# chansoopark98/Deep-Visual-SLAM

Hardware: AMD Instinct MI355X
Metric: VO training-step frames/sec (3-frame 640x480 snippets) (higher is better)
Workload: dtype f32; 1 GPU; configs[2]/[3]: full 4-scale photometric+smoothness loss, batch 12 per GPU, ResNet-18; per_gpu_batch=12, global_batch=12, num_scales=4, image=640x480, parallelism=dp1, streams=depth | pose | 2x weight-gradient, optimizer=fused Adam pass at lr 0: every step computes from the seeded weights, gpu_max_hw_queues=4

## Files before the change

deep-visual-slam_amd/csrc/conv_thin.hip:

```cpp
#include "conv_common.h"

#include <cstdlib>
#include <type_traits>

#ifndef THIN_DBG
#define THIN_DBG 0
#endif

namespace dvsconv {
namespace {

struct ThinParams {
    const float* x;
    const float* x2;
    const float* dy;
    const float* y;
    float* dw;
    float* dbias;
    int B, H, W, C1, C2, up, dact;
    int nseg, rows_per_wg, row_chunks;
};

template <int MT>
struct Acc {
    using type = typename std::conditional<MT == 32, f32x16, f32x4>::type;
};

template <int I, int N, class F>
__device__ __forceinline__ void static_for_thin(F&& f) {
    if constexpr (I < N) {
        f(std::integral_constant<int, I>{});
        static_for_thin<I + 1, N>(f);
    }
}

__device__ __forceinline__ f32x16 mma(float a, float b, f32x16 c) { return __builtin_amdgcn_mfma_f32_32x32x2f32(a, b, c, 0, 0, 0); }
__device__ __forceinline__ f32x4 mma(float a, float b, f32x4 c) { return __builtin_amdgcn_mfma_f32_16x16x4f32(a, b, c, 0, 0, 0); }

template <int MT, int CIN, int SEG>
__global__ __launch_bounds__(NT) void thin_wgrad_kernel(ThinParams p) {
    constexpr int KS = 64 / MT;
    constexpr int CT = CIN / MT;
    constexpr int NTILE = 9 * CT;
    constexpr int PWAVES = (MT == 16) ? 4 : 1;
    constexpr int TWAVES = 4 / PWAVES;
    constexpr int TPW = (NTILE + TWAVES - 1) / TWAVES;
    constexpr int PXW = SEG / PWAVES;
    constexpr int STEPS = PXW / KS;
    constexpr int CS = (MT == 16 && CIN % 32 == 0) ? CIN + 16 : CIN;
    constexpr int COLS = SEG + 2;
    constexpr int ROWF = COLS * CS;
    constexpr int XV = CIN / 4, ROW_VECS = COLS * XV, X_LOADS = (ROW_VECS + NT - 1) / NT;
    constexpr int DV = MT / 4, D_VECS = SEG * DV, D_LOADS = (D_VECS + NT - 1) / NT;
    static_assert(CIN % MT == 0 && SEG % (PWAVES * KS) == 0 && D_VECS % 64 == 0, "shape");
    using acc_t = typename Acc<MT>::type;
    constexpr int NR = (MT == 32) ? 16 : 4;

    __shared__ __attribute__((aligned(16))) float Ps[4 * ROWF];
    __shared__ __attribute__((aligned(16))) float Ds[2][SEG][MT];

    const int tid = threadIdx.x, lane = tid & 63;
    const int wave = __builtin_amdgcn_readfirstlane(tid >> 6);
    const int pw = wave / TWAVES, tw = wave % TWAVES;
    int lg = xcd_logical(blockIdx.x, gridDim.x, 1);
    const int chunk = lg % p.row_chunks;
    lg /= p.row_chunks;
    const int seg = lg % p.nseg, b = lg / p.nseg;
    const int oy_begin = chunk * p.rows_per_wg, oy_end = min(p.H, oy_begin + p.rows_per_wg);
    const int x0 = seg * SEG;
    const int Cout = MT, Ktot = 9 * CIN;
    const int H1 = p.up ? p.H >> 1 : p.H, W1 = p.up ? p.W >> 1 : p.W;

    int x_goff[X_LOADS], x_loff[X_LOADS];
    bool x_ok[X_LOADS], x_is2[X_LOADS];
#pragma unroll
    for (int j = 0; j < X_LOADS; ++j) {
        const int idx = tid + NT * j;
        x_ok[j] = idx < ROW_VECS;
        const int px = min(idx, ROW_VECS - 1) / XV, c = (min(idx, ROW_VECS - 1) % XV) * 4;
        const int sx = reflect_i(x0 - 1 + px, p.W);
        x_is2[j] = c >= p.C1;
        x_goff[j] = x_is2[j] ? sx * p.C2 + (c - p.C1) : (p.up ? sx >> 1 : sx) * p.C1 + c;
        x_loff[j] = px * CS + c;
    }
#ifdef THIN_NS
    constexpr int NS = THIN_NS;
#else
    constexpr int NS = 2;
#endif
    f32x4 rx[NS > 3 ? NS : 3][X_LOADS];
    auto load_row = [&](int pr, auto set) {
        constexpr int S = decltype(set)::value;
        const int sr = reflect_i(min(pr, p.H + 1) - 1, p.H);
        const float* r1 = p.x + ((size_t)b * H1 + (p.up ? sr >> 1 : sr)) * W1 * p.C1;
        const float* r2 = p.C2 > 0 ? p.x2 + ((size_t)b * p.H + sr) * p.W * p.C2 : r1;
#pragma unroll
        for (int j = 0; j < X_LOADS; ++j) rx[S][j] = *reinterpret_cast<const f32x4*>((x_is2[j] ? r2 : r1) + x_goff[j]);
    };
    auto store_row = [&](int pr, auto set) {
        constexpr int S = decltype(set)::value;
        float* dst = Ps + (pr & 3) * ROWF;
#pragma unroll
        for (int j = 0; j < X_LOADS; ++j)
            if (x_ok[j]) *reinterpret_cast<f32x4*>(dst + x_loff[j]) = rx[S][j];
    };

    f32x4 rd[NS][D_LOADS], ry[NS][D_LOADS], bsum = {0.f, 0.f, 0.f, 0.f};
    const int d_c = (tid % DV) * 4;
    const bool d_ok = tid < D_VECS;
    auto load_d = [&](int oy, auto set) {
        constexpr int S = decltype(set)::value;
        if (d_ok) {
#pragma unroll
            for (int j = 0; j < D_LOADS; ++j) {
                const size_t o = (((size_t)b * p.H + min(oy, p.H - 1)) * p.W + x0 + (tid + NT * j) / DV) * Cout + d_c;
                rd[S][j] = *reinterpret_cast<const f32x4*>(p.dy + o);
                if (p.dact) ry[S][j] = *reinterpret_cast<const f32x4*>(p.y + o);
            }
        }
    };
    auto store_d = [&](int buf, auto set) {
        constexpr int S = decltype(set)::value;
        if (d_ok) {
#pragma unroll
            for (int j = 0; j < D_LOADS; ++j) {
                f32x4 v = rd[S][j];
                if (p.dact == ACT_ELU) {
#pragma unroll
                    for (int e = 0; e < 4; ++e) v[e] = fmaf(v[e], fminf(ry[S][j][e], 0.f), v[e]);
                } else if (p.dact) {
#pragma unroll
                    for (int e = 0; e < 4; ++e) v[e] *= act_grad_from_out(ry[S][j][e], p.dact);
                }
                *reinterpret_cast<f32x4*>(&Ds[buf][(tid + NT * j) / DV][d_c]) = v;
                bsum += v;
            }
        }
    };

    const int col = lane % MT, kidx = lane / MT;
    int t_ky[TPW], t_off[TPW];
    bool t_ok[TPW];
#pragma unroll
    for (int i = 0; i < TPW; ++i) {
        const int q = tw + TWAVES * i;
        t_ok[i] = q < NTILE;
        const int qq = t_ok[i] ? q : 0;
        const int tap = qq / CT, ct = qq % CT;
        t_ky[i] = tap / 3;
        t_off[i] = (tap % 3) * CS + ct * MT;
    }
    const int b_lane = (pw * PXW + kidx) * CS + col;
    const int a_lane = (pw * PXW + kidx) * MT + col;

    acc_t acc[TPW];
#pragma unroll
    for (int i = 0; i < TPW; ++i)
#pragma unroll
        for (int r = 0; r < NR; ++r) acc[i][r] = 0.f;

    using S0 = std::integral_constant<int, 0>;
    if (oy_begin < oy_end) {
        static_for_thin<0, 3>([&](auto k) { load_row(oy_begin + k.value, k); });
        load_d(oy_begin, S0{});
        static_for_thin<0, 3>([&](auto k) { store_row(oy_begin + k.value, k); });
        store_d(0, S0{});
        static_for_thin<0, NS - 1>([&](auto k) {
            load_row(oy_begin + 3 + k.value, k);
            load_d(oy_begin + 1 + k.value, k);
        });
        for (int i = tid; i < ROWF; i += NT) Ps[((oy_begin + 3) & 3) * ROWF + i] = 0.f;
        for (int i = tid; i < SEG * MT; i += NT) (&Ds[1][0][0])[i] = 0.f;
    }
    __syncthreads();
    int buf = 0;
    auto stage = [&](int oy, auto set) {
        constexpr int S = decltype(set)::value;
        using Free = std::integral_constant<int, (S + NS - 1) % NS>;
        const bool more = oy + 1 < oy_end;
        if (oy + NS < oy_end && !(THIN_DBG & 1)) {
            load_row(oy + 2 + NS, Free{});
            load_d(oy + NS, Free{});
        }
        const float* Ab = &Ds[buf][0][0] + a_lane;
        const float* Bb[TPW];
#pragma unroll
        for (int i = 0; i < TPW; ++i) Bb[i] = Ps + ((oy + t_ky[i]) & 3) * ROWF + t_off[i] + b_lane;
        const float live = oy < oy_end ? 1.f : 0.f;
        float aq[2], bq[2][TPW];
        aq[0] = Ab[0];
#pragma unroll
        for (int i = 0; i < TPW; ++i) bq[0][i] = Bb[i][0];
#pragma unroll
        for (int t = 0; t < STEPS; ++t) {
            if (t + 1 < STEPS) {
                aq[(t + 1) & 1] = Ab[(t + 1) * KS * MT];
#pragma unroll
                for (int i = 0; i < TPW; ++i) bq[(t + 1) & 1][i] = Bb[i][(t + 1) * KS * CS];
            }
            __builtin_amdgcn_sched_barrier(0);
            const float a = aq[t & 1] * live;
            if constexpr (THIN_DBG & 2) {
#pragma unroll
                for (int i = 0; i < TPW; ++i) acc[i][0] += a * bq[t & 1][i];
            } else {
#pragma unroll
                for (int i = 0; i < TPW; ++i) acc[i] = mma(a, bq[t & 1][i], acc[i]);
            }
            __builtin_amdgcn_sched_barrier(0);
        }
        if (more && !(THIN_DBG & 4)) {
            store_row(oy + 3, set);
            store_d(buf ^ 1, set);
        }
        if (!(THIN_DBG & 8)) __syncthreads();
        buf ^= 1;
    };
#pragma unroll 1
    for (int oy = oy_begin; oy < oy_end; oy += NS) static_for_thin<0, NS>([&](auto k) { stage(oy + k.value, k); });

    if constexpr (PWAVES > 1) {
        static_assert(Cout * 9 * CIN <= 4 * ROWF, "dW fits the ring");
        float* sw = Ps;
        for (int i = tid; i < Cout * Ktot; i += NT) sw[i] = 0.f;
        __syncthreads();
#pragma unroll
        for (int i = 0; i < TPW; ++i) {
            if (!t_ok[i]) continue;
            const int q = tw + TWAVES * i;
            const int kk = (q / CT) * CIN + (q % CT) * MT + col;
#pragma unroll
            for (int r = 0; r < NR; ++r) atomicAdd(sw + (4 * (lane >> 4) + r) * Ktot + kk, acc[i][r]);
        }
        __syncthreads();
        constexpr int NW = Cout * 9 * CIN;
        const int rot = (int)((blockIdx.x * 7u) % (unsigned)(NW / NT)) * NT;
        for (int i = tid; i < NW; i += NT) {
            const int j = i + rot < NW ? i + rot : i + rot - NW;
            atomicAdd(p.dw + j, sw[j]);
        }
    } else {
#pragma unroll
        for (int i = 0; i < TPW; ++i) {
            if (!t_ok[i]) continue;
            const int q = tw + TWAVES * i;
            const int kk = (q / CT) * CIN + (q % CT) * MT + col;
#pragma unroll
            for (int r = 0; r < NR; ++r) {
                const int co = (MT == 32) ? (r & 3) + 8 * (r >> 2) + 4 * (lane >> 5) : 4 * (lane >> 4) + r;
                atomicAdd(p.dw + (size_t)co * Ktot + kk, acc[i][r]);
            }
        }
    }
    if (p.dbias) {
        float* sb = &Ds[0][0][0];
        if (tid < MT) sb[tid] = 0.f;
        __syncthreads();
        if (d_ok) {
#pragma unroll
            for (int e = 0; e < 4; ++e) atomicAdd(&sb[d_c + e], bsum[e]);
        }
        __syncthreads();
        if (tid < MT) atomicAdd(p.dbias + tid, sb[tid]);
    }
}

template <int MT, int CIN, int SEG>
void launch_thin(ThinParams p, hipStream_t st) {
    p.nseg = p.W / SEG;
    static const int slots = [] {
        int occ = 0, dev = 0, cus = 256;
        hipGetDevice(&dev);
        hipDeviceGetAttribute(&cus, hipDeviceAttributeMultiprocessorCount, dev);
        if (hipOccupancyMaxActiveBlocksPerMultiprocessor(&occ, thin_wgrad_kernel<MT, CIN, SEG>, NT, 0) != hipSuccess || occ < 1) occ = 1;
        return cus * occ;
    }();
    const int cols = p.B * p.nseg;
    int chunks = max(1, min(slots / cols, p.H / 8));
    p.rows_per_wg = (p.H + chunks - 1) / chunks;
    p.row_chunks = (p.H + p.rows_per_wg - 1) / p.rows_per_wg;
    dvs::ProfScope prof(dvs::SLOT_CONV_WGRAD, st);
    prof.work(2.0 * p.B * p.H * p.W * MT * 9.0 * CIN);
    hipLaunchKernelGGL((thin_wgrad_kernel<MT, CIN, SEG>), dim3(cols * p.row_chunks), dim3(NT), 0, st, p);
}


struct ThinFwdParams {
    const float* x;
    const float* w;
    const float* bias;
    float* y;
    int B, H, W, up, act;
    int nseg, rows_per_wg, row_chunks;
};

__device__ __forceinline__ float thin_act(float v, int act) {
    switch (act) {
        case ACT_RELU: return fmaxf(v, 0.f);
        case ACT_ELU: return v > 0.f ? v : __expf(v) - 1.f;
        case ACT_SIGMOID: return 1.f / (1.f + __expf(-v));
        default: return v;
    }
}

template <int CIN, int SEG>
__global__ __launch_bounds__(NT) void thin_fwd_kernel(ThinFwdParams p) {
    constexpr int CO = 16;
    constexpr int CS = CIN + 2;
    constexpr int COLS = SEG + 2, ROWF = COLS * CS;
    constexpr int XV = CIN / 4, ROW_VECS = COLS * XV, X_LOADS = (ROW_VECS + NT - 1) / NT;
    constexpr int PXW = SEG / 4, PT = PXW / 16;
    constexpr int C4 = CIN / 4, KSTEPS = 9 * C4;
    static_assert(PXW % 16 == 0 && (ROWF % 2) == 0, "shape");
    __shared__ __attribute__((aligned(16))) float Ps[4 * ROWF];

    const int tid = threadIdx.x, lane = tid & 63;
    const int wave = __builtin_amdgcn_readfirstlane(tid >> 6);
    int lg = xcd_logical(blockIdx.x, gridDim.x, 1);
    const int chunk = lg % p.row_chunks;
    lg /= p.row_chunks;
    const int seg = lg % p.nseg, b = lg / p.nseg;
    const int oy_begin = chunk * p.rows_per_wg, oy_end = min(p.H, oy_begin + p.rows_per_wg);
    const int x0 = seg * SEG;
    const int H1 = p.up ? p.H >> 1 : p.H, W1 = p.up ? p.W >> 1 : p.W;

    int x_goff[X_LOADS], x_loff[X_LOADS];
    bool x_ok[X_LOADS];
#pragma unroll
    for (int j = 0; j < X_LOADS; ++j) {
        const int idx = tid + NT * j;
        x_ok[j] = idx < ROW_VECS;
        const int px = min(idx, ROW_VECS - 1) / XV, c = (min(idx, ROW_VECS - 1) % XV) * 4;
        const int sx = reflect_i(x0 - 1 + px, p.W);
        x_goff[j] = (p.up ? sx >> 1 : sx) * CIN + c;
        x_loff[j] = px * CS + c;
    }
    f32x4 rx[X_LOADS];
    auto load_row_to = [&](int pr, f32x4 (&r)[X_LOADS]) {
        const int sr = reflect_i(pr - 1, p.H);
        const float* r1 = p.x + ((size_t)b * H1 + (p.up ? sr >> 1 : sr)) * W1 * CIN;
#pragma unroll
        for (int j = 0; j < X_LOADS; ++j) r[j] = *reinterpret_cast<const f32x4*>(r1 + x_goff[j]);
    };
    auto store_row_from = [&](int pr, const f32x4 (&r)[X_LOADS]) {
        float* dst = Ps + (pr & 3) * ROWF;
#pragma unroll
        for (int j = 0; j < X_LOADS; ++j)
            if (x_ok[j]) {
                float2* d2 = reinterpret_cast<float2*>(dst + x_loff[j]);
                d2[0] = float2{r[j][0], r[j][1]};
                d2[1] = float2{r[j][2], r[j][3]};
            }
    };
    auto load_row = [&](int pr) { load_row_to(pr, rx); };
    auto store_row = [&](int pr) { store_row_from(pr, rx); };

    const int n = lane & 15, kidx = lane >> 4;
    float wreg[KSTEPS];
#pragma unroll
    for (int s = 0; s < KSTEPS; ++s) wreg[s] = p.w[(size_t)n * (9 * CIN) + (s / C4) * CIN + (s % C4) * 4 + kidx];
    const float bv = p.bias ? p.bias[n] : 0.f;
    const int a_lane = (wave * PXW + n) * CS + kidx;

    if (oy_begin < oy_end) {
        f32x4 r0[X_LOADS], r1[X_LOADS];
        load_row_to(oy_begin, r0);
        load_row_to(oy_begin + 1, r1);
        load_row(oy_begin + 2);
        store_row_from(oy_begin, r0);
        store_row_from(oy_begin + 1, r1);
        store_row(oy_begin + 2);
    }
    __syncthreads();
#pragma unroll 1
    for (int oy = oy_begin; oy < oy_end; ++oy) {
        const bool more = oy + 1 < oy_end;
        if (more) load_row(oy + 3);
        const float* Ar[3];
#pragma unroll
        for (int ky = 0; ky < 3; ++ky) Ar[ky] = Ps + ((oy + ky) & 3) * ROWF + a_lane;
        f32x4 acc[PT];
#pragma unroll
        for (int t = 0; t < PT; ++t) acc[t] = f32x4{0.f, 0.f, 0.f, 0.f};
#pragma unroll
        for (int s = 0; s < KSTEPS; ++s) {
            const int tap = s / C4, c4 = s % C4, ky = tap / 3, kx = tap % 3;
#pragma unroll
            for (int t = 0; t < PT; ++t) acc[t] = mma(Ar[ky][(t * 16 + kx) * CS + c4 * 4], wreg[s], acc[t]);
        }
        float* yrow = p.y + (((size_t)b * p.H + oy) * p.W + x0 + wave * PXW + 4 * kidx) * CO + n;
#pragma unroll
        for (int t = 0; t < PT; ++t)
#pragma unroll
            for (int r = 0; r < 4; ++r) yrow[(t * 16 + r) * CO] = thin_act(acc[t][r] + bv, p.act);
        if (more) store_row(oy + 3);
        __syncthreads();
    }
}

template <int CIN, int SEG>
void launch_thin_fwd(ThinFwdParams p, hipStream_t st) {
    p.nseg = p.W / SEG;
    static const int slots = [] {
        int occ = 0, dev = 0, cus = 256;
        hipGetDevice(&dev);
        hipDeviceGetAttribute(&cus, hipDeviceAttributeMultiprocessorCount, dev);
        if (hipOccupancyMaxActiveBlocksPerMultiprocessor(&occ, thin_fwd_kernel<CIN, SEG>, NT, 0) != hipSuccess || occ < 1) occ = 1;
        return cus * occ;
    }();
    const int cols = p.B * p.nseg;
    int chunks = max(1, min(slots / cols, p.H / 8));
    p.rows_per_wg = (p.H + chunks - 1) / chunks;
    p.row_chunks = (p.H + p.rows_per_wg - 1) / p.rows_per_wg;
    dvs::ProfScope prof(dvs::SLOT_CONV_FWD, st);
    prof.work(2.0 * p.B * p.H * p.W * 16 * 9.0 * CIN);
    hipLaunchKernelGGL((thin_fwd_kernel<CIN, SEG>), dim3(cols * p.row_chunks), dim3(NT), 0, st, p);
}


struct ThinDgradParams {
    const float* dy;
    const float* y;
    const float* wt;
    float* dx;
    float* dx_skip;
    int B, H, W, dact, nout, C1;
    int nseg, rows_per_wg, row_chunks, nsplit;
};

template <int CK, int NTN, int SEG>
__device__ __forceinline__ void thin_dgrad_body(const ThinDgradParams& p) {
    constexpr int CS = CK + 2, C4 = CK / 4;
    constexpr int COLS = SEG + 2, ROWF = COLS * CS;
    constexpr int ROW_VECS = COLS * C4, X_LOADS = (ROW_VECS + NT - 1) / NT;
    constexpr int PXW = SEG / 4, PT = PXW / 16;
    static_assert(PXW % 16 == 0, "shape");
    __shared__ __attribute__((aligned(16))) float Ps[4 * ROWF];

    const int tid = threadIdx.x, lane = tid & 63;
    const int wave = __builtin_amdgcn_readfirstlane(tid >> 6);
    int lg = xcd_logical(blockIdx.x, gridDim.x, 1);
    const int split = lg % p.nsplit;
    lg /= p.nsplit;
    const int chunk = lg % p.row_chunks;
    lg /= p.row_chunks;
    const int seg = lg % p.nseg, b = lg / p.nseg;
    const int iy_begin = chunk * p.rows_per_wg, iy_end = min(p.H, iy_begin + p.rows_per_wg);
    const int x0 = seg * SEG;
    const int n_base = split * 16 * NTN;
    bool coarse[NTN];
    bool any_coarse = false, any_direct = false;
#pragma unroll
    for (int nt = 0; nt < NTN; ++nt) {
        coarse[nt] = n_base + nt * 16 < p.C1;
        any_coarse = any_coarse || coarse[nt];
        any_direct = any_direct || !coarse[nt];
    }

    int x_goff[X_LOADS], x_loff[X_LOADS];
    bool x_ok[X_LOADS], x_in[X_LOADS];
#pragma unroll
    for (int j = 0; j < X_LOADS; ++j) {
        const int idx = tid + NT * j;
        x_ok[j] = idx < ROW_VECS;
        const int e = min(idx, ROW_VECS - 1) / C4, c = (min(idx, ROW_VECS - 1) % C4) * 4;
        const int col = x0 - 1 + e;
        x_in[j] = (unsigned)col < (unsigned)p.W;
        x_goff[j] = clampi(col, p.W) * CK + c;
        x_loff[j] = e * CS + c;
    }
    constexpr int NS = (NTN == 3) ? 2 : 1;
    f32x4 rd[3][X_LOADS], ry[3][X_LOADS];
    const bool elu = p.dact == ACT_ELU;
    auto load_row = [&](int d, auto set) {
        constexpr int S = decltype(set)::value;
        const size_t ro = ((size_t)b * p.H + clampi(d, p.H)) * p.W * CK;
#pragma unroll
        for (int j = 0; j < X_LOADS; ++j) {
            rd[S][j] = *reinterpret_cast<const f32x4*>(p.dy + ro + x_goff[j]);
            if (p.dact) ry[S][j] = *reinterpret_cast<const f32x4*>(p.y + ro + x_goff[j]);
        }
    };
    auto store_row = [&](int d, auto set) {
        constexpr int S = decltype(set)::value;
        const bool row_in = (unsigned)d < (unsigned)p.H;
        float* dst = Ps + ((d + 1) & 3) * ROWF;
#pragma unroll
        for (int j = 0; j < X_LOADS; ++j)
            if (x_ok[j]) {
                f32x4 v = rd[S][j];
                const bool in = row_in && x_in[j];
#pragma unroll
                for (int e = 0; e < 4; ++e) {
                    const float g = elu ? fmaf(v[e], fminf(ry[S][j][e], 0.f), v[e]) : (p.dact ? v[e] * act_grad_from_out(ry[S][j][e], p.dact) : v[e]);
                    v[e] = in ? g : 0.f;
                }
                float2* d2 = reinterpret_cast<float2*>(dst + x_loff[j]);
                d2[0] = float2{v[0], v[1]};
                d2[1] = float2{v[2], v[3]};
            }
    };

    const int n = lane & 15, kidx = lane >> 4;
    float wreg[NTN][9 * C4];
#pragma unroll
    for (int nt = 0; nt < NTN; ++nt)
#pragma unroll
        for (int s = 0; s < 9 * C4; ++s)
            wreg[nt][s] = p.wt[((size_t)(n_base + nt * 16 + n) * 9 + s / C4) * CK + (s % C4) * 4 + kidx];
    const int a_lane = (wave * PXW + n) * CS + kidx;
    const int wseg = min(SEG, p.W - x0);
    const bool edge_l = seg == 0 && wave == 0, edge_r = seg == p.nseg - 1 && wave == wseg / PXW - 1;
    const bool wave_live = wave * PXW < wseg;
    const int fold_l = ((n == 1) ? 1 : 0) * CS + kidx;
    const int fold_r = ((n == 14) ? wseg : wseg + 1) * CS + kidx;

    f32x4 acc[PT][NTN];
    auto zero_acc = [&]() {
#pragma unroll
        for (int t = 0; t < PT; ++t)
#pragma unroll
            for (int nt = 0; nt < NTN; ++nt) acc[t][nt] = f32x4{0.f, 0.f, 0.f, 0.f};
    };
    zero_acc();

    using S0 = std::integral_constant<int, 0>;
    if (iy_begin < iy_end) {
        static_for_thin<0, 3>([&](auto k) { load_row(iy_begin - 1 + k.value, k); });
        static_for_thin<0, 3>([&](auto k) { store_row(iy_begin - 1 + k.value, k); });
        static_for_thin<0, NS - 1>([&](auto k) { load_row(iy_begin + 2 + k.value, k); });
    }
    __syncthreads();
    auto stage = [&](int iy, auto set) {
        constexpr int S = decltype(set)::value;
        using Free = std::integral_constant<int, (S + NS - 1) % NS>;
        const bool more = iy + 1 < iy_end;
        if (iy + NS < iy_end && !(THIN_DBG & 1)) load_row(iy + 1 + NS, Free{});
        auto lda = [&](float (&a)[PT][C4], const float* row, int kx) {
#pragma unroll
            for (int t = 0; t < PT; ++t)
#pragma unroll
                for (int c4 = 0; c4 < C4; ++c4) a[t][c4] = row[a_lane + (t * 16 + 2 - kx) * CS + c4 * 4];
            if (kx == 0 && edge_l) {
#pragma unroll
                for (int c4 = 0; c4 < C4; ++c4) a[0][c4] += row[fold_l + c4 * 4];
            }
            if (kx == 2 && edge_r) {
#pragma unroll
                for (int c4 = 0; c4 < C4; ++c4) a[PT - 1][c4] += row[fold_r + c4 * 4];
            }
        };
        auto mfmas = [&](const float (&a)[PT][C4], int tap) {
#pragma unroll
            for (int c4 = 0; c4 < C4; ++c4)
#pragma unroll
                for (int t = 0; t < PT; ++t)
#pragma unroll
                    for (int nt = 0; nt < NTN; ++nt) {
                        if constexpr (THIN_DBG & 2) acc[t][nt][0] += a[t][c4] * wreg[nt][tap * C4 + c4];
                        else acc[t][nt] = mma(a[t][c4], wreg[nt][tap * C4 + c4], acc[t][nt]);
                    }
        };
        auto taps = [&](const float* row, int ky) {
#pragma unroll
            for (int kx = 0; kx < 3; ++kx) {
                float a[PT][C4];
                lda(a, row, kx);
                mfmas(a, ky * 3 + kx);
            }
        };
        const float* rows[3];
#pragma unroll
        for (int ky = 0; ky < 3; ++ky) rows[ky] = Ps + ((iy + 2 - ky) & 3) * ROWF;
        float abuf[2][PT][C4];
        lda(abuf[0], rows[0], 0);
        static_for_thin<0, 9>([&](auto ic) {
            constexpr int I = decltype(ic)::value;
            if constexpr (I + 1 < 9) lda(abuf[(I + 1) & 1], rows[(I + 1) / 3], (I + 1) % 3);
            __builtin_amdgcn_sched_barrier(0);
            mfmas(abuf[I & 1], I);
            __builtin_amdgcn_sched_barrier(0);
        });
        if (iy == 1) {
            const float* row = Ps + 1 * ROWF;
            taps(row, 0);
        }
        if (iy == p.H - 2) {
            const float* row = Ps + (p.H & 3) * ROWF;
            taps(row, 2);
        }
        if (any_coarse && (iy & 1) && wave_live && !(THIN_DBG & 16)) {
            float* orow = p.dx + (((size_t)b * (p.H >> 1) + (iy >> 1)) * (p.W >> 1) + ((x0 + wave * PXW + 4 * kidx) >> 1)) * p.C1 +
                          n_base + n;
#pragma unroll
            for (int nt = 0; nt < NTN; ++nt)
                if (coarse[nt]) {
#pragma unroll
                    for (int t = 0; t < PT; ++t) {
                        orow[(size_t)(t * 8 + 0) * p.C1 + nt * 16] = acc[t][nt][0] + acc[t][nt][1];
                        orow[(size_t)(t * 8 + 1) * p.C1 + nt * 16] = acc[t][nt][2] + acc[t][nt][3];
                        acc[t][nt] = f32x4{0.f, 0.f, 0.f, 0.f};
                    }
                }
        }
        if (any_direct && wave_live && !(THIN_DBG & 16)) {
            const int cs = p.nout - p.C1;
            float* base = p.C1 > 0 ? p.dx_skip : p.dx;
            float* orow = base + (((size_t)b * p.H + iy) * p.W + x0 + wave * PXW + 4 * kidx) * cs + (n_base - p.C1) + n;
#pragma unroll
            for (int nt = 0; nt < NTN; ++nt)
                if (!coarse[nt]) {
#pragma unroll
                    for (int t = 0; t < PT; ++t) {
#pragma unroll
                        for (int r = 0; r < 4; ++r) orow[(size_t)(t * 16 + r) * cs + nt * 16] = acc[t][nt][r];
                        acc[t][nt] = f32x4{0.f, 0.f, 0.f, 0.f};
                    }
                }
        }
        if (more && !(THIN_DBG & 4)) store_row(iy + 2, set);
        if (!(THIN_DBG & 8)) __syncthreads();
    };
#pragma unroll 1
    for (int iy = iy_begin; iy < iy_end; iy += NS)
        static_for_thin<0, NS>([&](auto k) {
            if (k.value == 0 || iy + k.value < iy_end) stage(iy + k.value, k);
        });
}

template <int CK, int NTN, int SEG>
__global__ __launch_bounds__(NT) void thin_dgrad_kernel(ThinDgradParams p) {
    thin_dgrad_body<CK, NTN, SEG>(p);
}
template <int CK, int NTN, int SEG>
__global__ __launch_bounds__(NT) __attribute__((amdgpu_waves_per_eu(1, 1))) void thin_dgrad_kernel_w1(ThinDgradParams p) {
    thin_dgrad_body<CK, NTN, SEG>(p);
}

template <int CK, int NTN, int SEG, bool W1 = false>
void launch_thin_dgrad(ThinDgradParams p, hipStream_t st) {
    auto kern = W1 ? thin_dgrad_kernel_w1<CK, NTN, SEG> : thin_dgrad_kernel<CK, NTN, SEG>;
    p.nseg = (p.W + SEG - 1) / SEG;
    p.nsplit = p.nout / (16 * NTN);
    static const int slots = [] {
        int occ = 0, dev = 0, cus = 256;
        hipGetDevice(&dev);
        hipDeviceGetAttribute(&cus, hipDeviceAttributeMultiprocessorCount, dev);
        auto k = W1 ? thin_dgrad_kernel_w1<CK, NTN, SEG> : thin_dgrad_kernel<CK, NTN, SEG>;
        if (hipOccupancyMaxActiveBlocksPerMultiprocessor(&occ, k, NT, 0) != hipSuccess || occ < 1) occ = 1;
        return cus * occ;
    }();
    const int cols = p.B * p.nseg * p.nsplit;
    int chunks = max(1, min(slots / cols, p.H / 8));
    p.rows_per_wg = ((p.H + chunks - 1) / chunks + 1) & ~1;
    p.row_chunks = (p.H + p.rows_per_wg - 1) / p.rows_per_wg;
    dvs::ProfScope prof(dvs::SLOT_CONV_DGRAD, st);
    prof.work(2.0 * p.B * p.H * p.W * CK * 9.0 * p.nout);
    hipLaunchKernelGGL(kern, dim3(cols * p.row_chunks), dim3(NT), 0, st, p);
}

}

bool thin_wgrad_shape(const ConvShape& s, const InXform& t) {
    static const bool enabled = [] { const char* e = getenv("DVS_CONV_THIN"); return !(e && e[0] == '0'); }();
    if (!enabled || s.kh != 3 || s.kw != 3 || s.stride != 1 || s.pad != 1 || s.pad_mode != PAD_REFLECT || t.in_scale) return false;
    if (s.H < 8 || (t.x2 && ((s.H | s.W) & 1))) return false;
    const int C1 = t.x2 != nullptr ? t.C1 : s.Cin;
    if (C1 <= 0 || (C1 & 3) || s.Cin - C1 < 0) return false;
    return (s.Cout == 32 && s.Cin == 96 && s.W % 32 == 0) || (s.Cout == 32 && s.Cin == 64 && s.W % 32 == 0) ||
           (s.Cout == 16 && s.Cin == 32 && s.W % 64 == 0) || (s.Cout == 16 && s.Cin == 16 && s.W % 128 == 0);
}

bool thin_wgrad(const float* x, const float* dy, float* dw, float* dbias, const ConvShape& s, const InXform& t,
                hipStream_t st) {
    if (!thin_wgrad_shape(s, t)) return false;
    ThinParams p{};
    p.x = x; p.dy = dy; p.y = t.aux; p.dw = dw; p.dbias = dbias;
    p.B = s.B; p.H = s.H; p.W = s.W; p.dact = t.dact;
    p.up = t.x2 != nullptr;
    p.C1 = p.up ? t.C1 : s.Cin;
    p.C2 = s.Cin - p.C1;
    p.x2 = p.C2 > 0 ? t.x2 : nullptr;
    if (p.C1 <= 0 || (p.C1 & 3) || p.C2 < 0) return false;
    if (s.Cout == 32 && s.Cin == 96 && s.W % 32 == 0) launch_thin<32, 96, 32>(p, st);
    else if (s.Cout == 32 && s.Cin == 64 && s.W % 32 == 0) launch_thin<32, 64, 32>(p, st);
    else if (s.Cout == 16 && s.Cin == 32 && s.W % 64 == 0) launch_thin<16, 32, 64>(p, st);
    else if (s.Cout == 16 && s.Cin == 16 && s.W % 128 == 0) launch_thin<16, 16, 128>(p, st);
    else return false;
    return true;
}

}

namespace dvsconv {

bool thin_fwd(const float* x, const float* w, const float* bias, float* y, const ConvShape& s, const InXform& t, int act,
              hipStream_t st) {
    static const bool enabled = [] { const char* e = getenv("DVS_CONV_THIN"); return !(e && e[0] == '0'); }();
    if (!enabled || s.kh != 3 || s.kw != 3 || s.stride != 1 || s.pad != 1 || s.pad_mode != PAD_REFLECT || t.in_scale) return false;
    if (s.Cout != 16 || s.H < 8 || (t.x2 && (t.C1 != s.Cin || ((s.H | s.W) & 1)))) return false;
    ThinFwdParams p{};
    p.x = x; p.w = w; p.bias = bias; p.y = y;
    p.B = s.B; p.H = s.H; p.W = s.W; p.up = t.x2 != nullptr; p.act = act;
    if (s.Cin == 16 && s.W % 128 == 0) launch_thin_fwd<16, 128>(p, st);
    else if (s.Cin == 32 && s.W % 64 == 0) launch_thin_fwd<32, 64>(p, st);
    else return false;
    return true;
}

}

namespace dvsconv {

bool thin_dgrad(const float* dy, const float* wt, float* dx, const float* y_out, int dact, int B, int H, int W, int Cin,
                int Cout, int split_c1, float* dx_skip, hipStream_t st) {
    static const bool enabled = [] { const char* e = getenv("DVS_CONV_THIN"); return !(e && e[0] == '0'); }();
    if (!enabled || H < 8) return false;
    if (split_c1 > 0 && (((H | W) & 1) || (split_c1 < Cin && !dx_skip))) return false;
    ThinDgradParams p{};
    p.dy = dy; p.y = y_out; p.wt = wt; p.dx = dx; p.dx_skip = dx_skip; p.B = B; p.H = H; p.W = W; p.dact = dact;
    p.nout = Cin; p.C1 = split_c1;
    if (Cout == 16 && Cin == 16 && split_c1 == 16 && W % 128 == 0) launch_thin_dgrad<16, 1, 128>(p, st);
    else if (Cout == 16 && Cin == 32 && split_c1 == 0 && W % 64 == 0) launch_thin_dgrad<16, 2, 64>(p, st);
    else if (Cout == 32 && Cin % 48 == 0 && Cin <= 192 && split_c1 % 16 == 0 && W % 64 == 0)
        launch_thin_dgrad<32, 3, 64, true>(p, st);
    else if (Cout == 32 && Cin % 32 == 0 && Cin <= 128 && split_c1 % 16 == 0 && (W % 64 == 0 || (W % 16 == 0 && W > 64)))
        launch_thin_dgrad<32, 2, 64>(p, st);
    else return false;
    return true;
}

}
```

Measured before the change: 1534 frames/s.

## Fold nearest-upsample into 3x3 conv via polyphase 2x2 kernels for fwd/dgrad/wgrad

For the 16->16 channel 3x3 conv that consumes a 2x nearest-upsampled input, adds polyphase kernels that work on the low-resolution tensor. The forward pass computes each of the four output phases with pre-summed 2x2 weights, cutting the 9 taps to 4 per phase and reading only the half-resolution input. Matching dgrad and wgrad phase kernels fold the upsample adjoint and the weight summation the same way, with reflect-edge fixups. The new paths are on by default and can be disabled through DVS_UPSAMPLE_PHASE; edge folding and the pad handling add correctness risk.

```diff
diff --git a/deep-visual-slam_amd/csrc/conv_thin.hip b/deep-visual-slam_amd/csrc/conv_thin.hip
--- a/deep-visual-slam_amd/csrc/conv_thin.hip
+++ b/deep-visual-slam_amd/csrc/conv_thin.hip
@@ -415,6 +415,356 @@
     dvs::ProfScope prof(dvs::SLOT_CONV_FWD, st);
     prof.work(2.0 * p.B * p.H * p.W * 16 * 9.0 * CIN);
     hipLaunchKernelGGL((thin_fwd_kernel<CIN, SEG>), dim3(cols * p.row_chunks), dim3(NT), 0, st, p);
+}
+
+
+__host__ __device__ constexpr int phase_lo(int par, int a) { return par == 0 ? (a == 0 ? 0 : 1) : (a == 0 ? 0 : 2); }
+__host__ __device__ constexpr int phase_hi(int par, int a) { return par == 0 ? (a == 0 ? 0 : 2) : (a == 0 ? 1 : 2); }
+
+template <int SEG>
+__global__ __launch_bounds__(NT) void thin_fwd_phase_kernel(ThinFwdParams p) {
+    constexpr int CIN = 16, CO = 16, C4 = CIN / 4;
+    constexpr int CS = CIN + 2;
+    constexpr int LSEG = SEG / 2, COLS = LSEG + 2, ROWF = COLS * CS;
+    constexpr int XV = CIN / 4, ROW_VECS = COLS * XV, X_LOADS = (ROW_VECS + NT - 1) / NT;
+    constexpr int PXW = LSEG / 4;
+    static_assert(PXW == 16, "one 16-pixel tile per wave and column parity");
+    __shared__ __attribute__((aligned(16))) float Ps[4 * ROWF];
+
+    const int tid = threadIdx.x, lane = tid & 63;
+    const int wave = __builtin_amdgcn_readfirstlane(tid >> 6);
+    int lg = xcd_logical(blockIdx.x, gridDim.x, 1);
+    const int chunk = lg % p.row_chunks;
+    lg /= p.row_chunks;
+    const int seg = lg % p.nseg, b = lg / p.nseg;
+    const int h = p.H >> 1, w = p.W >> 1;
+    const int i_begin = chunk * p.rows_per_wg, i_end = min(h, i_begin + p.rows_per_wg);
+    const int xl0 = seg * LSEG;
+
+    int x_goff[X_LOADS], x_loff[X_LOADS];
+    bool x_ok[X_LOADS];
+#pragma unroll
+    for (int j = 0; j < X_LOADS; ++j) {
+        const int idx = tid + NT * j;
+        x_ok[j] = idx < ROW_VECS;
+        const int e = min(idx, ROW_VECS - 1) / XV, c = (min(idx, ROW_VECS - 1) % XV) * 4;
+        x_goff[j] = clampi(xl0 - 1 + e, w) * CIN + c;
+        x_loff[j] = e * CS + c;
+    }
+    f32x4 rx[X_LOADS];
+    auto load_row_to = [&](int pr, f32x4 (&r)[X_LOADS]) {
+        const float* r1 = p.x + ((size_t)b * h + clampi(pr - 1, h)) * w * CIN;
+#pragma unroll
+        for (int j = 0; j < X_LOADS; ++j) r[j] = *reinterpret_cast<const f32x4*>(r1 + x_goff[j]);
+    };
+    auto store_row_from = [&](int pr, const f32x4 (&r)[X_LOADS]) {
+        float* dst = Ps + (pr & 3) * ROWF;
+#pragma unroll
+        for (int j = 0; j < X_LOADS; ++j)
+            if (x_ok[j]) {
+                float2* d2 = reinterpret_cast<float2*>(dst + x_loff[j]);
+                d2[0] = float2{r[j][0], r[j][1]};
+                d2[1] = float2{r[j][2], r[j][3]};
+            }
+    };
+
+    const int n = lane & 15, kidx = lane >> 4;
+    float wp[2][2][2][2][C4];
+    {
+        float w3[9][C4];
+#pragma unroll
+        for (int tap = 0; tap < 9; ++tap)
+#pragma unroll
+            for (int c4 = 0; c4 < C4; ++c4) w3[tap][c4] = p.w[(size_t)n * (9 * CIN) + tap * CIN + c4 * 4 + kidx];
+#pragma unroll
+        for (int py = 0; py < 2; ++py)
+#pragma unroll
+            for (int px = 0; px < 2; ++px)
+#pragma unroll
+                for (int a = 0; a < 2; ++a)
+#pragma unroll
+                    for (int bb = 0; bb < 2; ++bb)
+#pragma unroll
+                        for (int c4 = 0; c4 < C4; ++c4) {
+                            float s = 0.f;
+#pragma unroll
+                            for (int ky = phase_lo(py, a); ky <= phase_hi(py, a); ++ky)
+#pragma unroll
+                                for (int kx = phase_lo(px, bb); kx <= phase_hi(px, bb); ++kx) s += w3[ky * 3 + kx][c4];
+                            wp[py][px][a][bb][c4] = s;
+                        }
+    }
+    const float bv = p.bias ? p.bias[n] : 0.f;
+    const int a_lane = (wave * PXW + n) * CS + kidx;
+
+    if (i_begin < i_end) {
+        f32x4 r0[X_LOADS], r1[X_LOADS];
+        load_row_to(i_begin, r0);
+        load_row_to(i_begin + 1, r1);
+        load_row_to(i_begin + 2, rx);
+        store_row_from(i_begin, r0);
+        store_row_from(i_begin + 1, r1);
+        store_row_from(i_begin + 2, rx);
+    }
+    __syncthreads();
+#pragma unroll 1
+    for (int i = i_begin; i < i_end; ++i) {
+        const bool more = i + 1 < i_end;
+        if (more) load_row_to(i + 3, rx);
+        float av[3][3][C4];
+#pragma unroll
+        for (int r = 0; r < 3; ++r) {
+            const float* row = Ps + ((i + r) & 3) * ROWF + a_lane;
+#pragma unroll
+            for (int d = 0; d < 3; ++d)
+#pragma unroll
+                for (int c4 = 0; c4 < C4; ++c4) av[r][d][c4] = row[d * CS + c4 * 4];
+        }
+        __builtin_amdgcn_sched_barrier(0);
+        f32x4 acc[2][2];
+#pragma unroll
+        for (int py = 0; py < 2; ++py)
+#pragma unroll
+            for (int px = 0; px < 2; ++px) acc[py][px] = f32x4{0.f, 0.f, 0.f, 0.f};
+#pragma unroll
+        for (int a = 0; a < 2; ++a)
+#pragma unroll
+            for (int bb = 0; bb < 2; ++bb)
+#pragma unroll
+                for (int c4 = 0; c4 < C4; ++c4)
+#pragma unroll
+                    for (int py = 0; py < 2; ++py)
+#pragma unroll
+                        for (int px = 0; px < 2; ++px)
+                            acc[py][px] = mma(av[py + a][px + bb][c4], wp[py][px][a][bb][c4], acc[py][px]);
+        float* yrow = p.y + (((size_t)b * p.H + 2 * i) * p.W + 2 * (xl0 + wave * PXW + 4 * kidx)) * CO + n;
+#pragma unroll
+        for (int py = 0; py < 2; ++py)
+#pragma unroll
+            for (int r = 0; r < 4; ++r)
+#pragma unroll
+                for (int px = 0; px < 2; ++px)
+                    yrow[((size_t)py * p.W + 2 * r + px) * CO] = thin_act(acc[py][px][r] + bv, p.act);
+        if (more) store_row_from(i + 3, rx);
+        __syncthreads();
+    }
+}
+
+template <int SEG>
+void launch_thin_fwd_phase(ThinFwdParams p, hipStream_t st) {
+    p.nseg = p.W / SEG;
+    static const int slots = [] {
+        int occ = 0, dev = 0, cus = 256;
+        hipGetDevice(&dev);
+        hipDeviceGetAttribute(&cus, hipDeviceAttributeMultiprocessorCount, dev);
+        if (hipOccupancyMaxActiveBlocksPerMultiprocessor(&occ, thin_fwd_phase_kernel<SEG>, NT, 0) != hipSuccess || occ < 1) occ = 1;
+        return cus * occ;
+    }();
+    const int cols = p.B * p.nseg, h = p.H >> 1;
+    int chunks = max(1, min(slots / cols, h / 4));
+    p.rows_per_wg = (h + chunks - 1) / chunks;
+    p.row_chunks = (h + p.rows_per_wg - 1) / p.rows_per_wg;
+    dvs::ProfScope prof(dvs::SLOT_CONV_FWD, st);
+    prof.work(2.0 * p.B * p.H * p.W * 16 * 9.0 * 16);
+    hipLaunchKernelGGL((thin_fwd_phase_kernel<SEG>), dim3(cols * p.row_chunks), dim3(NT), 0, st, p);
+}
+
+bool upsample_phase_enabled() {
+    static const bool enabled = [] { const char* e = getenv("DVS_UPSAMPLE_PHASE"); return !(e && e[0] == '0'); }();
+    return enabled;
+}
+
+
+template <int SEG>
+__global__ __launch_bounds__(NT) void thin_wgrad_phase_kernel(ThinParams p) {
+    constexpr int MT = 16, CIN = 16, KS = 4;
+    constexpr int LSEG = SEG / 2, COLS = LSEG + 2, CS = CIN, ROWF = COLS * CS;
+    constexpr int XV = CIN / 4, ROW_VECS = COLS * XV, X_LOADS = (ROW_VECS + NT - 1) / NT;
+    constexpr int DV = MT / 4, D_VECS = SEG * DV, D_LOADS = D_VECS / NT;
+    constexpr int PXW = LSEG / 4, STEPS = PXW / KS;
+    constexpr int PLANE = (LSEG + 2) * MT;
+    constexpr int Ktot = 9 * CIN;
+    static_assert(D_VECS % NT == 0 && PXW % KS == 0 && MT * Ktot <= 4 * ROWF, "shape");
+
+    __shared__ __attribute__((aligned(16))) float Ps[4 * ROWF];
+    __shared__ __attribute__((aligned(16))) float Ds[2][2 * PLANE];
+
+    const int tid = threadIdx.x, lane = tid & 63;
+    const int pw = __builtin_amdgcn_readfirstlane(tid >> 6);
+    int lg = xcd_logical(blockIdx.x, gridDim.x, 1);
+    const int chunk = lg % p.row_chunks;
+    lg /= p.row_chunks;
+    const int seg = lg % p.nseg, b = lg / p.nseg;
+    const int h = p.H >> 1, w = p.W >> 1;
+    const int i_begin = chunk * p.rows_per_wg, i_end = min(h, i_begin + p.rows_per_wg);
+    const int x0 = seg * SEG, xl0 = seg * LSEG;
+
+    int x_goff[X_LOADS], x_loff[X_LOADS];
+    bool x_ok[X_LOADS];
+#pragma unroll
+    for (int j = 0; j < X_LOADS; ++j) {
+        const int idx = tid + NT * j;
+        x_ok[j] = idx < ROW_VECS;
+        const int e = min(idx, ROW_VECS - 1) / XV, c = (min(idx, ROW_VECS - 1) % XV) * 4;
+        x_goff[j] = clampi(xl0 - 1 + e, w) * CIN + c;
+        x_loff[j] = e * CS + c;
+    }
+    f32x4 rx[3][X_LOADS];
+    auto load_row = [&](int pr, auto set) {
+        constexpr int S = decltype(set)::value;
+        const float* r1 = p.x + ((size_t)b * h + clampi(pr - 1, h)) * w * CIN;
+#pragma unroll
+        for (int j = 0; j < X_LOADS; ++j) rx[S][j] = *reinterpret_cast<const f32x4*>(r1 + x_goff[j]);
+    };
+    auto store_row = [&](int pr, auto set) {
+        constexpr int S = decltype(set)::value;
+        float* dst = Ps + (pr & 3) * ROWF;
+#pragma unroll
+        for (int j = 0; j < X_LOADS; ++j)
+            if (x_ok[j]) *reinterpret_cast<f32x4*>(dst + x_loff[j]) = rx[S][j];
+    };
+
+    f32x4 rd[2][D_LOADS], ry[2][D_LOADS], bsum = {0.f, 0.f, 0.f, 0.f};
+    const int d_c = (tid % DV) * 4;
+    auto load_d = [&](int oy, auto set) {
+        constexpr int S = decltype(set)::value;
+#pragma unroll
+        for (int j = 0; j < D_LOADS; ++j) {
+            const size_t o = (((size_t)b * p.H + oy) * p.W + x0 + (tid + NT * j) / DV) * MT + d_c;
+            rd[S][j] = *reinterpret_cast<const f32x4*>(p.dy + o);
+            if (p.dact) ry[S][j] = *reinterpret_cast<const f32x4*>(p.y + o);
+        }
+    };
+    auto store_d = [&](int buf, auto set) {
+        constexpr int S = decltype(set)::value;
+#pragma unroll
+        for (int j = 0; j < D_LOADS; ++j) {
+            f32x4 v = rd[S][j];
+            if (p.dact == ACT_ELU) {
+#pragma unroll
+                for (int e = 0; e < 4; ++e) v[e] = fmaf(v[e], fminf(ry[S][j][e], 0.f), v[e]);
+            } else if (p.dact) {
+#pragma unroll
+                for (int e = 0; e < 4; ++e) v[e] *= act_grad_from_out(ry[S][j][e], p.dact);
+            }
+            const int pix = (tid + NT * j) / DV;
+            *reinterpret_cast<f32x4*>(&Ds[buf][(pix & 1) * PLANE + (pix >> 1) * MT + d_c]) = v;
+            bsum += v;
+        }
+    };
+
+    const int col = lane % MT, kidx = lane / MT;
+    const int b_lane = (pw * PXW + kidx) * CS + col;
+    const int a_lane = (pw * PXW + kidx) * MT + col;
+
+    f32x4 acc[2][2][2][2];
+#pragma unroll
+    for (int i = 0; i < 16; ++i) (&acc[0][0][0][0])[i] = f32x4{0.f, 0.f, 0.f, 0.f};
+
+    using S0 = std::integral_constant<int, 0>;
+    using S1 = std::integral_constant<int, 1>;
+    if (i_begin < i_end) {
+        static_for_thin<0, 3>([&](auto k) { load_row(i_begin + k.value, k); });
+        load_d(2 * i_begin, S0{});
+        static_for_thin<0, 3>([&](auto k) { store_row(i_begin + k.value, k); });
+        store_d(0, S0{});
+        load_d(2 * i_begin + 1, S0{});
+        if (i_begin + 1 < i_end) load_d(2 * i_begin + 2, S1{});
+    }
+    __syncthreads();
+    auto stage = [&](int i, auto parity) {
+        constexpr int PY = decltype(parity)::value;
+        using Set = std::integral_constant<int, PY>;
+        const bool more = i + 1 < i_end;
+        if (PY == 0 || more) store_d(PY ^ 1, Set{});
+        if (i + 1 + PY < i_end) load_d(2 * i + 3 + PY, Set{});
+        if (PY == 0 && more) load_row(i + 3, S0{});
+        const float* Ab = &Ds[PY][0] + a_lane;
+        const float* Bb[2];
+#pragma unroll
+        for (int r = 0; r < 2; ++r) Bb[r] = Ps + ((i + PY + r) & 3) * ROWF + b_lane;
+        float aq[2][2], bq[2][2][3];
+        auto ld = [&](int s, int t) {
+#pragma unroll
+            for (int px = 0; px < 2; ++px) aq[s][px] = Ab[px * PLANE + t * KS * MT];
+#pragma unroll
+            for (int r = 0; r < 2; ++r)
+#pragma unroll
+                for (int d = 0; d < 3; ++d) bq[s][r][d] = Bb[r][(t * KS + d) * CS];
+        };
+        ld(0, 0);
+#pragma unroll
+        for (int t = 0; t < STEPS; ++t) {
+            if (t + 1 < STEPS) ld((t + 1) & 1, t + 1);
+            __builtin_amdgcn_sched_barrier(0);
+#pragma unroll
+            for (int a = 0; a < 2; ++a)
+#pragma unroll
+                for (int bb = 0; bb < 2; ++bb)
+#pragma unroll
+                    for (int px = 0; px < 2; ++px)
+                        acc[PY][px][a][bb] = mma(aq[t & 1][px], bq[t & 1][a][px + bb], acc[PY][px][a][bb]);
+            __builtin_amdgcn_sched_barrier(0);
+        }
+        if (PY == 1 && more) store_row(i + 3, S0{});
+        __syncthreads();
+    };
+#pragma unroll 1
+    for (int i = i_begin; i < i_end; ++i) {
+        stage(i, S0{});
+        stage(i, S1{});
+    }
+
+    float* sw = Ps;
+    for (int i = tid; i < MT * Ktot; i += NT) sw[i] = 0.f;
+    __syncthreads();
+#pragma unroll
+    for (int ky = 0; ky < 3; ++ky)
+#pragma unroll
+        for (int kx = 0; kx < 3; ++kx) {
+            f32x4 s = {0.f, 0.f, 0.f, 0.f};
+#pragma unroll
+            for (int py = 0; py < 2; ++py)
+#pragma unroll
+                for (int px = 0; px < 2; ++px) s += acc[py][px][ky > phase_hi(py, 0) ? 1 : 0][kx > phase_hi(px, 0) ? 1 : 0];
+#pragma unroll
+            for (int r = 0; r < 4; ++r) atomicAdd(sw + (4 * (lane >> 4) + r) * Ktot + (ky * 3 + kx) * CIN + col, s[r]);
+        }
+    __syncthreads();
+    constexpr int NW = MT * Ktot;
+    const int rot = (int)((blockIdx.x * 7u) % (unsigned)(NW / NT)) * NT;
+    for (int i = tid; i < NW; i += NT) {
+        const int j = i + rot < NW ? i + rot : i + rot - NW;
+        atomicAdd(p.dw + j, sw[j]);
+    }
+    if (p.dbias) {
+        float* sb = &Ds[0][0];
+        if (tid < MT) sb[tid] = 0.f;
+        __syncthreads();
+#pragma unroll
+        for (int e = 0; e < 4; ++e) atomicAdd(&sb[d_c + e], bsum[e]);
+        __syncthreads();
+        if (tid < MT) atomicAdd(p.dbias + tid, sb[tid]);
+    }
+}
+
+template <int SEG>
+void launch_thin_phase(ThinParams p, hipStream_t st) {
+    p.nseg = p.W / SEG;
+    static const int slots = [] {
+        int occ = 0, dev = 0, cus = 256;
+        hipGetDevice(&dev);
+        hipDeviceGetAttribute(&cus, hipDeviceAttributeMultiprocessorCount, dev);
+        if (hipOccupancyMaxActiveBlocksPerMultiprocessor(&occ, thin_wgrad_phase_kernel<SEG>, NT, 0) != hipSuccess || occ < 1) occ = 1;
+        return cus * occ;
+    }();
+    const int cols = p.B * p.nseg, h = p.H >> 1;
+    int chunks = max(1, min(slots / cols, h / 4));
+    p.rows_per_wg = (h + chunks - 1) / chunks;
+    p.row_chunks = (h + p.rows_per_wg - 1) / p.rows_per_wg;
+    dvs::ProfScope prof(dvs::SLOT_CONV_WGRAD, st);
+    prof.work(2.0 * p.B * p.H * p.W * 16 * 9.0 * 16);
+    hipLaunchKernelGGL((thin_wgrad_phase_kernel<SEG>), dim3(cols * p.row_chunks), dim3(NT), 0, st, p);
 }
 
 
@@ -659,6 +1009,189 @@
     hipLaunchKernelGGL(kern, dim3(cols * p.row_chunks), dim3(NT), 0, st, p);
 }
 
+template <int SEG>
+__global__ __launch_bounds__(NT) __attribute__((amdgpu_waves_per_eu(3, 3))) void thin_dgrad_phase_kernel(ThinDgradParams p) {
+    constexpr int CK = 16, CS = CK + 2, C4 = CK / 4;
+    constexpr int COLS = SEG + 2, ROWF = COLS * CS;
+    constexpr int X_LOADS = SEG * C4 / NT;
+    constexpr int LSEG = SEG / 2, PXW = LSEG / 4;
+    static_assert(PXW == 16 && SEG * C4 % NT == 0 && 2 * CK <= 64, "one 16-pixel tile per wave; the halo is staged by half a wave");
+    __shared__ __attribute__((aligned(16))) float Ps[4 * ROWF];
+
+    const int tid = threadIdx.x, lane = tid & 63;
+    const int wave = __builtin_amdgcn_readfirstlane(tid >> 6);
+    int lg = xcd_logical(blockIdx.x, gridDim.x, 1);
+    const int chunk = lg % p.row_chunks;
+    lg /= p.row_chunks;
+    const int seg = lg % p.nseg, b = lg / p.nseg;
+    const int h = p.H >> 1, w = p.W >> 1;
+    const int r_begin = chunk * p.rows_per_wg, r_end = min(h, r_begin + p.rows_per_wg);
+    const int x0 = seg * SEG;
+
+    const int x_goff = (x0 + tid / C4) * CK + (tid % C4) * 4;
+    const int x_loff = (1 + tid / C4) * CS + (tid % C4) * 4;
+    const bool h_ok = tid < 2 * CK;
+    const int h_e = tid < CK ? 0 : SEG + 1, h_col = x0 - 1 + h_e;
+    const bool h_in = (unsigned)h_col < (unsigned)p.W;
+    const int h_goff = clampi(h_col, p.W) * CK + (tid & (CK - 1)), h_loff = h_e * CS + (tid & (CK - 1));
+    f32x4 rd[2][X_LOADS], ry[2][X_LOADS];
+    float hd[2], hy[2];
+    const bool elu = p.dact == ACT_ELU;
+    auto dz = [&](float d, float y) {
+        return elu ? fmaf(d, fminf(y, 0.f), d) : (p.dact ? d * act_grad_from_out(y, p.dact) : d);
+    };
+    auto load_row = [&](int d, auto set) {
+        constexpr int S = decltype(set)::value;
+        const size_t ro = ((size_t)b * p.H + clampi(d, p.H)) * p.W * CK;
+#pragma unroll
+        for (int j = 0; j < X_LOADS; ++j) {
+            rd[S][j] = *reinterpret_cast<const f32x4*>(p.dy + ro + x_goff + j * (NT / C4) * CK);
+            if (p.dact) ry[S][j] = *reinterpret_cast<const f32x4*>(p.y + ro + x_goff + j * (NT / C4) * CK);
+        }
+        if (h_ok) {
+            hd[S] = p.dy[ro + h_goff];
+            if (p.dact) hy[S] = p.y[ro + h_goff];
+        }
+    };
+    auto store_row = [&](int d, auto set) {
+        constexpr int S = decltype(set)::value;
+        const bool row_in = (unsigned)d < (unsigned)p.H;
+        float* dst = Ps + ((d + 1) & 3) * ROWF;
+#pragma unroll
+        for (int j = 0; j < X_LOADS; ++j) {
+            f32x4 v = rd[S][j];
+#pragma unroll
+            for (int e = 0; e < 4; ++e) v[e] = row_in ? dz(v[e], p.dact ? ry[S][j][e] : 0.f) : 0.f;
+            float2* d2 = reinterpret_cast<float2*>(dst + x_loff + j * (NT / C4) * CS);
+            d2[0] = float2{v[0], v[1]};
+            d2[1] = float2{v[2], v[3]};
+        }
+        if (h_ok) dst[h_loff] = (row_in && h_in) ? dz(hd[S], p.dact ? hy[S] : 0.f) : 0.f;
+    };
+
+    const int n = lane & 15, kidx = lane >> 4;
+    float wp[2][2][2][2][C4];
+    {
+        float w3[9][C4];
+#pragma unroll
+        for (int tap = 0; tap < 9; ++tap)
+#pragma unroll
+            for (int c4 = 0; c4 < C4; ++c4) w3[tap][c4] = p.wt[((size_t)n * 9 + tap) * CK + c4 * 4 + kidx];
+#pragma unroll
+        for (int py = 0; py < 2; ++py)
+#pragma unroll
+            for (int px = 0; px < 2; ++px)
+#pragma unroll
+                for (int a = 0; a < 2; ++a)
+#pragma unroll
+                    for (int bb = 0; bb < 2; ++bb)
+#pragma unroll
+                        for (int c4 = 0; c4 < C4; ++c4) {
+                            float s = 0.f;
+#pragma unroll
+                            for (int ky = phase_lo(py, a); ky <= phase_hi(py, a); ++ky)
+#pragma unroll
+                                for (int kx = phase_lo(px, bb); kx <= phase_hi(px, bb); ++kx) s += w3[ky * 3 + kx][c4];
+                            wp[py][px][a][bb][c4] = s;
+                        }
+    }
+    const int a_lane = (wave * 2 * PXW + 2 * n) * CS + kidx;
+    const bool edge_l = seg == 0 && wave == 0, edge_r = seg == p.nseg - 1 && wave == 3;
+    const int fold_l = ((n == 0) ? 1 : 0) * CS + kidx;
+    const int fold_r = ((n == 15) ? SEG : SEG + 1) * CS + kidx;
+
+    using S0 = std::integral_constant<int, 0>;
+    using S1 = std::integral_constant<int, 1>;
+    if (r_begin < r_end) {
+        load_row(2 * r_begin - 1, S0{});
+        load_row(2 * r_begin, S1{});
+        store_row(2 * r_begin - 1, S0{});
+        store_row(2 * r_begin, S1{});
+        load_row(2 * r_begin + 1, S0{});
+        load_row(2 * r_begin + 2, S1{});
+        store_row(2 * r_begin + 1, S0{});
+        store_row(2 * r_begin + 2, S1{});
+    }
+    __syncthreads();
+#pragma unroll 1
+    for (int r = r_begin; r < r_end; ++r) {
+        const bool more = r + 1 < r_end;
+        if (more) {
+            load_row(2 * r + 3, S0{});
+            load_row(2 * r + 4, S1{});
+        }
+        f32x4 acc[2] = {f32x4{0.f, 0.f, 0.f, 0.f}, f32x4{0.f, 0.f, 0.f, 0.f}};
+        auto lda = [&](float (&av)[2][2][C4], int d) {
+            const float* row = Ps + ((d + 1) & 3) * ROWF;
+#pragma unroll
+            for (int px = 0; px < 2; ++px)
+#pragma unroll
+                for (int bb = 0; bb < 2; ++bb)
+#pragma unroll
+                    for (int c4 = 0; c4 < C4; ++c4) av[px][bb][c4] = row[a_lane + (3 - px - 2 * bb) * CS + c4 * 4];
+            if (edge_l) {
+#pragma unroll
+                for (int c4 = 0; c4 < C4; ++c4) av[0][0][c4] += row[fold_l + c4 * 4];
+            }
+            if (edge_r) {
+#pragma unroll
+                for (int c4 = 0; c4 < C4; ++c4) av[1][1][c4] += row[fold_r + c4 * 4];
+            }
+        };
+        auto mfmas = [&](const float (&av)[2][2][C4], auto pyc, auto ac) {
+            constexpr int PY = decltype(pyc)::value, A = decltype(ac)::value;
+#pragma unroll
+            for (int c4 = 0; c4 < C4; ++c4)
+#pragma unroll
+                for (int bb = 0; bb < 2; ++bb)
+#pragma unroll
+                    for (int px = 0; px < 2; ++px) acc[px] = mma(av[px][bb][c4], wp[PY][px][A][bb][c4], acc[px]);
+        };
+        float av0[2][2][C4], av1[2][2][C4];
+        lda(av0, 2 * r - 1);
+        lda(av1, 2 * r);
+        __builtin_amdgcn_sched_barrier(0);
+        mfmas(av0, S1{}, S1{});
+        mfmas(av1, S0{}, S1{});
+        if (r == 0) mfmas(av1, S0{}, S0{});
+        __builtin_amdgcn_sched_barrier(0);
+        __syncthreads();
+        lda(av0, 2 * r + 1);
+        lda(av1, 2 * r + 2);
+        __builtin_amdgcn_sched_barrier(0);
+        if (more) {
+            store_row(2 * r + 3, S0{});
+            store_row(2 * r + 4, S1{});
+        }
+        mfmas(av0, S1{}, S0{});
+        if (r == h - 1) mfmas(av0, S1{}, S1{});
+        mfmas(av1, S0{}, S0{});
+        float* orow = p.dx + (((size_t)b * h + r) * w + (x0 >> 1) + wave * PXW + 4 * kidx) * CK + n;
+#pragma unroll
+        for (int i = 0; i < 4; ++i) orow[i * CK] = acc[0][i] + acc[1][i];
+    }
+}
+
+template <int SEG>
+void launch_thin_dgrad_phase(ThinDgradParams p, hipStream_t st) {
+    p.nseg = p.W / SEG;
+    p.nsplit = 1;
+    static const int slots = [] {
+        int occ = 0, dev = 0, cus = 256;
+        hipGetDevice(&dev);
+        hipDeviceGetAttribute(&cus, hipDeviceAttributeMultiprocessorCount, dev);
+        if (hipOccupancyMaxActiveBlocksPerMultiprocessor(&occ, thin_dgrad_phase_kernel<SEG>, NT, 0) != hipSuccess || occ < 1) occ = 1;
+        return cus * occ;
+    }();
+    const int cols = p.B * p.nseg, h = p.H >> 1;
+    int chunks = max(1, min(slots / cols, h / 4));
+    p.rows_per_wg = (h + chunks - 1) / chunks;
+    p.row_chunks = (h + p.rows_per_wg - 1) / p.rows_per_wg;
+    dvs::ProfScope prof(dvs::SLOT_CONV_DGRAD, st);
+    prof.work(2.0 * p.B * p.H * p.W * 16 * 9.0 * 16);
+    hipLaunchKernelGGL((thin_dgrad_phase_kernel<SEG>), dim3(cols * p.row_chunks), dim3(NT), 0, st, p);
+}
+
 }
 
 bool thin_wgrad_shape(const ConvShape& s, const InXform& t) {
@@ -685,8 +1218,10 @@
     if (s.Cout == 32 && s.Cin == 96 && s.W % 32 == 0) launch_thin<32, 96, 32>(p, st);
     else if (s.Cout == 32 && s.Cin == 64 && s.W % 32 == 0) launch_thin<32, 64, 32>(p, st);
     else if (s.Cout == 16 && s.Cin == 32 && s.W % 64 == 0) launch_thin<16, 32, 64>(p, st);
-    else if (s.Cout == 16 && s.Cin == 16 && s.W % 128 == 0) launch_thin<16, 16, 128>(p, st);
-    else return false;
+    else if (s.Cout == 16 && s.Cin == 16 && s.W % 128 == 0) {
+        if (p.up && p.C2 == 0 && upsample_phase_enabled()) launch_thin_phase<128>(p, st);
+        else launch_thin<16, 16, 128>(p, st);
+    } else return false;
     return true;
 }
 
@@ -702,8 +1237,10 @@
     ThinFwdParams p{};
     p.x = x; p.w = w; p.bias = bias; p.y = y;
     p.B = s.B; p.H = s.H; p.W = s.W; p.up = t.x2 != nullptr; p.act = act;
-    if (s.Cin == 16 && s.W % 128 == 0) launch_thin_fwd<16, 128>(p, st);
-    else if (s.Cin == 32 && s.W % 64 == 0) launch_thin_fwd<32, 64>(p, st);
+    if (s.Cin == 16 && s.W % 128 == 0) {
+        if (p.up && upsample_phase_enabled()) launch_thin_fwd_phase<128>(p, st);
+        else launch_thin_fwd<16, 128>(p, st);
+    } else if (s.Cin == 32 && s.W % 64 == 0) launch_thin_fwd<32, 64>(p, st);
     else return false;
     return true;
 }
@@ -720,8 +1257,10 @@
     ThinDgradParams p{};
     p.dy = dy; p.y = y_out; p.wt = wt; p.dx = dx; p.dx_skip = dx_skip; p.B = B; p.H = H; p.W = W; p.dact = dact;
     p.nout = Cin; p.C1 = split_c1;
-    if (Cout == 16 && Cin == 16 && split_c1 == 16 && W % 128 == 0) launch_thin_dgrad<16, 1, 128>(p, st);
-    else if (Cout == 16 && Cin == 32 && split_c1 == 0 && W % 64 == 0) launch_thin_dgrad<16, 2, 64>(p, st);
+    if (Cout == 16 && Cin == 16 && split_c1 == 16 && W % 128 == 0) {
+        if (upsample_phase_enabled()) launch_thin_dgrad_phase<128>(p, st);
+        else launch_thin_dgrad<16, 1, 128>(p, st);
+    } else if (Cout == 16 && Cin == 32 && split_c1 == 0 && W % 64 == 0) launch_thin_dgrad<16, 2, 64>(p, st);
     else if (Cout == 32 && Cin % 48 == 0 && Cin <= 192 && split_c1 % 16 == 0 && W % 64 == 0)
         launch_thin_dgrad<32, 3, 64, true>(p, st);
     else if (Cout == 32 && Cin % 32 == 0 && Cin <= 128 && split_c1 % 16 == 0 && (W % 64 == 0 || (W % 16 == 0 && W > 64)))
```

New measurement: 1542 frames/s (median of 6 runs). No clear change (+0.5%).
